# William-wAng618/roboticAttack

Hardware: AMD Instinct MI355X
Metric: attack-steps/sec (bs=64, 3x50x50 patch, OpenVLA-7B) (higher is better)
Workload: dtype bf16; 1 GPU; UADA_wrapper_ddp inner step: bs=64/rank (global 64), patch 3,50,50, geometry=True, maskidx=[0]; OpenVLA-7B shape, random init; u8 frames resident in HBM; global_batch=64, parallelism=dp1, regions=weak, visible_gpus=1, labelled_rows_per_rank=128, tunableop_entries_loaded_min_over_ranks=173

## Files before the change

### roboticattack_amd/csrc/vaa_attention.hip

```cpp
#include "vaa_common.h"

#include <cstdlib>
#include <mutex>

#include "../../include/vaa_model_ops.h"

namespace vaa {

typedef short v4s __attribute__((ext_vector_type(4)));
typedef short v8s __attribute__((ext_vector_type(8)));
typedef float v4f __attribute__((ext_vector_type(4)));
typedef __attribute__((address_space(3))) v4s* lds_v4s_ptr;

struct AttnStr {
    long b, t, h;
};

struct AttnFwdArgs {
    const uint16_t *q, *k, *v;
    uint16_t* o;
    float* lse;
    AttnStr sq, sk, sv, so;
    const int32_t* cu;
    int B, H, T, hd;
    float scale_log2;
};

struct SeqInfo {
    int T;
    long tok0;
    bool packed;
};
__device__ __forceinline__ SeqInfo seq_info(const int32_t* cu, int b, int Tmax) {
    SeqInfo si;
    si.packed = cu != nullptr;
    si.tok0 = si.packed ? cu[b] : 0;
    si.T = si.packed ? cu[b + 1] - cu[b] : Tmax;
    return si;
}
__device__ __forceinline__ long row_base(const AttnStr& st, const SeqInfo& si, int b, int h) {
    return (si.packed ? si.tok0 * st.t : (long)b * st.b) + (long)h * st.h;
}

constexpr int kTile = 64;

__device__ __forceinline__ float fast_exp2(float x) { return __builtin_amdgcn_exp2f(x); }

__device__ __forceinline__ v4s lds_tr16(const uint16_t* p) {
    return __builtin_amdgcn_ds_read_tr16_b64_v4i16((lds_v4s_ptr)(p));
}

__device__ __forceinline__ v8s cat8(v4s lo, v4s hi) { return __builtin_shufflevector(lo, hi, 0, 1, 2, 3, 4, 5, 6, 7); }

typedef __bf16 bf2 __attribute__((ext_vector_type(2)));
typedef float f2 __attribute__((ext_vector_type(2)));

__device__ __forceinline__ uint32_t cvt_pk_bf16(float lo, float hi) {
    const bf2 r = __builtin_convertvector((f2){lo, hi}, bf2);
    return *reinterpret_cast<const uint32_t*>(&r);
}

__device__ __forceinline__ v8s pack8(v4f a, v4f b) {
    uint4 r;
    r.x = cvt_pk_bf16(a[0], a[1]);
    r.y = cvt_pk_bf16(a[2], a[3]);
    r.z = cvt_pk_bf16(b[0], b[1]);
    r.w = cvt_pk_bf16(b[2], b[3]);
    return *reinterpret_cast<v8s*>(&r);
}

typedef unsigned int v4u __attribute__((ext_vector_type(4)));

__device__ __forceinline__ __amdgpu_buffer_rsrc_t slice_rsrc(const uint16_t* base, long st, int T, int hd) {
    return __builtin_amdgcn_make_buffer_rsrc((void*)base, 0, (int)((((long)T - 1) * st + hd) * 2), 0x00020000);
}

template <int HDP>
struct TileRegs {
    static constexpr int kChunks = kTile * (HDP / 8) / 256;
    v4u r[kChunks];
    __device__ __forceinline__ void load(__amdgpu_buffer_rsrc_t rs, int st_bytes, int row0) {
#pragma unroll
        for (int it = 0; it < kChunks; ++it) {
            const int ch = threadIdx.x + it * 256;
            const int row = ch / (HDP / 8), cc = ch % (HDP / 8);
            r[it] = __builtin_amdgcn_raw_buffer_load_b128(rs, (row0 + row) * st_bytes + cc * 16, 0, 0);
        }
    }
    __device__ __forceinline__ void store(uint16_t* lds, int stride) const {
#pragma unroll
        for (int it = 0; it < kChunks; ++it) {
            const int ch = threadIdx.x + it * 256;
            const int row = ch / (HDP / 8), cc = ch % (HDP / 8);
            *reinterpret_cast<v4u*>(lds + row * stride + cc * 8) = r[it];
        }
    }
};

__device__ __forceinline__ bool block_to_pair(int nblk, int npairs, int& pair, int& blk, bool late_first = true) {
    const int bid = blockIdx.x, xcd = bid & 7, slot = bid >> 3;
    pair = (slot / nblk) * 8 + xcd;
    blk = late_first ? nblk - 1 - (slot % nblk) : slot % nblk;
    return pair < npairs;
}

template <int KS, int NT, bool CAUSAL, int G>
__global__ __launch_bounds__(256) void attn_fwd_kernel(AttnFwdArgs a) {
    constexpr int HDP = KS * 32;
    constexpr int SK = HDP + 8;
    constexpr int SV = HDP + 16;
    constexpr int QB = kTile * G, QW = 16 * G;
    __shared__ __attribute__((aligned(16))) uint16_t sK[kTile * SK];
    __shared__ __attribute__((aligned(16))) uint16_t sV[kTile * SV];

    const int nqb = (a.T + QB - 1) / QB;
    int pair, qb;
    if (!block_to_pair(nqb, a.B * a.H, pair, qb)) return;
    const int b = pair / a.H, h = pair - b * a.H;
    const SeqInfo si = seq_info(a.cu, b, a.T);
    const int T = si.T;
    if (qb * QB >= T) return;
    const int tid = threadIdx.x, lane = tid & 63, wv = tid >> 6, c = lane & 15, g = lane >> 4;
    const int q0 = qb * QB + wv * QW;

    const uint16_t* qp = a.q + row_base(a.sq, si, b, h);
    const uint16_t* kp = a.k + row_base(a.sk, si, b, h);
    const uint16_t* vp = a.v + row_base(a.sv, si, b, h);

    v8s qf[G][KS];
#pragma unroll
    for (int j = 0; j < G; ++j) {
        const int q = q0 + 16 * j + c;
#pragma unroll
        for (int ks = 0; ks < KS; ++ks) {
            const int d0 = ks * 32 + g * 8;
            uint4 r = make_uint4(0, 0, 0, 0);
            if (q < T && d0 < a.hd) r = *reinterpret_cast<const uint4*>(qp + (long)q * a.sq.t + d0);
            qf[j][ks] = *reinterpret_cast<v8s*>(&r);
        }
    }

    const int kend = CAUSAL ? min(T, (qb + 1) * QB) : T;
    const int ntile = (kend + kTile - 1) / kTile;

    v4f acc[G][NT];
    float m[G], lsum[G];
#pragma unroll
    for (int j = 0; j < G; ++j) {
#pragma unroll
        for (int nt = 0; nt < NT; ++nt) acc[j][nt] = (v4f){0.f, 0.f, 0.f, 0.f};
        m[j] = -INFINITY;
        lsum[j] = 0.0f;
    }

    const __amdgpu_buffer_rsrc_t krs = slice_rsrc(kp, a.sk.t, T, a.hd), vrs = slice_rsrc(vp, a.sv.t, T, a.hd);
    const int kst = (int)a.sk.t * 2, vst = (int)a.sv.t * 2;
    TileRegs<HDP> rk, rv;
    rk.load(krs, kst, 0);
    rv.load(vrs, vst, 0);
    for (int kt = 0; kt < ntile; ++kt) {
        __syncthreads();
        rk.store(sK, SK);
        rv.store(sV, SV);
        __syncthreads();
        if (kt + 1 < ntile) {
            rk.load(krs, kst, (kt + 1) * kTile);
            rv.load(vrs, vst, (kt + 1) * kTile);
        }
        const int key0 = kt * kTile;
        if (CAUSAL && key0 > q0 + QW - 1) continue;

        v4f st[G][4];
#pragma unroll
        for (int rp = 0; rp < 2; ++rp) {
            v8s kfr[2][KS];
#pragma unroll
            for (int rl = 0; rl < 2; ++rl)
#pragma unroll
                for (int ks = 0; ks < KS; ++ks) kfr[rl][ks] = *reinterpret_cast<const v8s*>(&sK[((2 * rp + rl) * 16 + c) * SK + ks * 32 + g * 8]);
#pragma unroll
            for (int j = 0; j < G; ++j)
#pragma unroll
                for (int rl = 0; rl < 2; ++rl) {
                    v4f t = (v4f){0.f, 0.f, 0.f, 0.f};
#pragma unroll
                    for (int ks = 0; ks < KS; ++ks) t = __builtin_amdgcn_mfma_f32_16x16x32_bf16(kfr[rl][ks], qf[j][ks], t, 0, 0, 0);
                    st[j][2 * rp + rl] = t;
                }
        }
#pragma unroll
        for (int j = 0; j < G; ++j) {
            const int qj0 = q0 + 16 * j, q = qj0 + c;
            const bool need_mask = (key0 + kTile > T) || (CAUSAL && key0 + kTile - 1 > qj0);
            if (need_mask) {
#pragma unroll
                for (int rt = 0; rt < 4; ++rt)
#pragma unroll
                    for (int r = 0; r < 4; ++r) {
                        const int key = key0 + rt * 16 + g * 4 + r;
                        if (key >= T || (CAUSAL && key > q)) st[j][rt][r] = -INFINITY;
                    }
            }
            float mx = -INFINITY;
#pragma unroll
            for (int rt = 0; rt < 4; ++rt)
#pragma unroll
                for (int r = 0; r < 4; ++r) mx = fmaxf(mx, st[j][rt][r]);
            mx = fmaxf(mx, __shfl_xor(mx, 16, 64));
            mx = fmaxf(mx, __shfl_xor(mx, 32, 64));
            const float mn = fmaxf(m[j], mx * a.scale_log2);
            const float mu = (mn == -INFINITY) ? 0.0f : mn;
            const float alpha = fast_exp2(m[j] - mu);
            m[j] = mn;
            float ps = 0.0f;
#pragma unroll
            for (int rt = 0; rt < 4; ++rt)
#pragma unroll
                for (int r = 0; r < 4; ++r) {
                    const float p = fast_exp2(__builtin_fmaf(st[j][rt][r], a.scale_log2, -mu));
                    st[j][rt][r] = p;
                    ps += p;
                }
            lsum[j] = lsum[j] * alpha + ps;
#pragma unroll
            for (int nt = 0; nt < NT; ++nt) acc[j][nt] *= alpha;
        }
#pragma unroll
        for (int half = 0; half < 2; ++half) {
            const uint16_t* vrow = &sV[(half * 32 + 4 * g + (c >> 2)) * SV + (c & 3) * 4];
            v8s vfr[NT];
#pragma unroll
            for (int nt = 0; nt < NT; ++nt) vfr[nt] = cat8(lds_tr16(vrow + nt * 16), lds_tr16(vrow + 16 * SV + nt * 16));
#pragma unroll
            for (int j = 0; j < G; ++j) {
                const v8s pf = pack8(st[j][2 * half], st[j][2 * half + 1]);
#pragma unroll
                for (int nt = 0; nt < NT; ++nt) acc[j][nt] = __builtin_amdgcn_mfma_f32_16x16x32_bf16(vfr[nt], pf, acc[j][nt], 0, 0, 0);
            }
        }
    }
#pragma unroll
    for (int j = 0; j < G; ++j) {
        const int q = q0 + 16 * j + c;
        float ls = lsum[j];
        ls += __shfl_xor(ls, 16, 64);
        ls += __shfl_xor(ls, 32, 64);
        if (q < T) {
            const float inv = ls > 0.0f ? 1.0f / ls : 0.0f;
            uint16_t* op = a.o + row_base(a.so, si, b, h) + (long)q * a.so.t;
#pragma unroll
            for (int nt = 0; nt < NT; ++nt) {
                const int d0 = nt * 16 + g * 4;
                if (d0 < a.hd) {
                    uint2 w;
                    w.x = cvt_pk_bf16(acc[j][nt][0] * inv, acc[j][nt][1] * inv);
                    w.y = cvt_pk_bf16(acc[j][nt][2] * inv, acc[j][nt][3] * inv);
                    *reinterpret_cast<uint2*>(op + d0) = w;
                }
            }
            if (g == 0) a.lse[((long)b * a.H + h) * a.T + q] = (m[j] + __builtin_log2f(ls)) * 0.69314718055994531f;
        }
    }
}

struct AttnBwdArgs {
    const uint16_t *q, *k, *v, *o, *dout;
    const float* lse;
    float* dsum;
    uint16_t *dq, *dk, *dv;
    AttnStr sq, sk, sv, so, sdo, sdq, sdk, sdv;
    const int32_t* cu;
    const float *rope_cos, *rope_sin;
    int B, H, T, hd;
    float scale, scale_log2;
};

template <int NT>
__device__ __forceinline__ void store_grad_row(uint16_t* op, const v4f (&acc)[NT], float scale, int g, int hd, const float* cosr, const float* sinr) {
    if (cosr) {
#pragma unroll
        for (int nt = 0; nt < NT / 2; ++nt) {
            const int d0 = nt * 16 + g * 4;
            const float4 c4 = *reinterpret_cast<const float4*>(cosr + d0), s4 = *reinterpret_cast<const float4*>(sinr + d0);
            const float cs[4] = {c4.x, c4.y, c4.z, c4.w}, sn[4] = {s4.x, s4.y, s4.z, s4.w};
            float o1[4], o2[4];
#pragma unroll
            for (int r = 0; r < 4; ++r) {
                const float g1 = acc[nt][r] * scale, g2 = acc[nt + NT / 2][r] * scale;
                o1[r] = g1 * cs[r] + g2 * sn[r];
                o2[r] = g2 * cs[r] - g1 * sn[r];
            }
            uint2 w;
            w.x = cvt_pk_bf16(o1[0], o1[1]); w.y = cvt_pk_bf16(o1[2], o1[3]);
            *reinterpret_cast<uint2*>(op + d0) = w;
            w.x = cvt_pk_bf16(o2[0], o2[1]); w.y = cvt_pk_bf16(o2[2], o2[3]);
            *reinterpret_cast<uint2*>(op + d0 + NT * 8) = w;
        }
        return;
    }
#pragma unroll
    for (int nt = 0; nt < NT; ++nt) {
        const int d0 = nt * 16 + g * 4;
        if (d0 < hd) {
            uint2 w;
            w.x = cvt_pk_bf16(acc[nt][0] * scale, acc[nt][1] * scale);
            w.y = cvt_pk_bf16(acc[nt][2] * scale, acc[nt][3] * scale);
            *reinterpret_cast<uint2*>(op + d0) = w;
        }
    }
}

template <int KS>
__device__ __forceinline__ void load_row_frags(v8s (&f)[KS], const uint16_t* row, bool valid, int g, int hd) {
#pragma unroll
    for (int ks = 0; ks < KS; ++ks) {
        const int d0 = ks * 32 + g * 8;
        uint4 r = make_uint4(0, 0, 0, 0);
        if (valid && d0 < hd) r = *reinterpret_cast<const uint4*>(row + d0);
        f[ks] = *reinterpret_cast<v8s*>(&r);
    }
}

__device__ __forceinline__ float bf_lo(uint32_t w) { return __uint_as_float(w << 16); }
__device__ __forceinline__ float bf_hi(uint32_t w) { return __uint_as_float(w & 0xffff0000u); }

template <int KS>
__device__ __forceinline__ void load_tile_frags(v8s (&af)[KS], const uint16_t* tile, int stride, int rt, int c, int g) {
#pragma unroll
    for (int ks = 0; ks < KS; ++ks) af[ks] = *reinterpret_cast<const v8s*>(&tile[(rt * 16 + c) * stride + ks * 32 + g * 8]);
}
template <int KS>
__device__ __forceinline__ v4f frag_dot(const v8s (&af)[KS], const v8s (&bf)[KS]) {
    v4f acc = (v4f){0.f, 0.f, 0.f, 0.f};
#pragma unroll
    for (int ks = 0; ks < KS; ++ks) acc = __builtin_amdgcn_mfma_f32_16x16x32_bf16(af[ks], bf[ks], acc, 0, 0, 0);
    return acc;
}

template <int KS, int NT, bool CAUSAL, int G>
__global__ __launch_bounds__(256) void attn_bwd_dq_kernel(AttnBwdArgs a) {
    constexpr int HDP = KS * 32;
    constexpr int SK = HDP + 16, SV = HDP + 8;
    constexpr int QB = kTile * G, QW = 16 * G;
    __shared__ __attribute__((aligned(16))) uint16_t sK[kTile * SK];
    __shared__ __attribute__((aligned(16))) uint16_t sV[kTile * SV];

    const int nqb = (a.T + QB - 1) / QB;
    int pair, qb;
    if (!block_to_pair(nqb, a.B * a.H, pair, qb)) return;
    const int b = pair / a.H, h = pair - b * a.H;
    const SeqInfo si = seq_info(a.cu, b, a.T);
    const int T = si.T;
    if (qb * QB >= T) return;
    const int tid = threadIdx.x, lane = tid & 63, wv = tid >> 6, c = lane & 15, g = lane >> 4;
    const int q0 = qb * QB + wv * QW;

    const uint16_t* kp = a.k + row_base(a.sk, si, b, h);
    const uint16_t* vp = a.v + row_base(a.sv, si, b, h);
    v8s qf[G][KS], dof[G][KS];
    float Dq[G], lse2[G];
#pragma unroll
    for (int j = 0; j < G; ++j) {
        const int q = q0 + 16 * j + c;
        const bool qv = q < T;
        load_row_frags<KS>(qf[j], a.q + row_base(a.sq, si, b, h) + (long)q * a.sq.t, qv, g, a.hd);
        load_row_frags<KS>(dof[j], a.dout + row_base(a.sdo, si, b, h) + (long)q * a.sdo.t, qv, g, a.hd);
        float dq_ = 0.0f;
        v8s of[KS];
        load_row_frags<KS>(of, a.o + row_base(a.so, si, b, h) + (long)q * a.so.t, qv, g, a.hd);
#pragma unroll
        for (int ks = 0; ks < KS; ++ks)
#pragma unroll
            for (int e = 0; e < 8; ++e) dq_ += bf16_bits_to_f32((uint16_t)of[ks][e]) * bf16_bits_to_f32((uint16_t)dof[j][ks][e]);
        dq_ += __shfl_xor(dq_, 16, 64);
        dq_ += __shfl_xor(dq_, 32, 64);
        Dq[j] = dq_;
        const long rowid = ((long)b * a.H + h) * a.T + q;
        if (qv && g == 0) a.dsum[rowid] = dq_;
        lse2[j] = qv ? a.lse[rowid] * 1.4426950408889634f : INFINITY;
    }

    const int kend = CAUSAL ? min(T, (qb + 1) * QB) : T;
    const int ntile = (kend + kTile - 1) / kTile;
    v4f acc[G][NT];
#pragma unroll
    for (int j = 0; j < G; ++j)
#pragma unroll
        for (int nt = 0; nt < NT; ++nt) acc[j][nt] = (v4f){0.f, 0.f, 0.f, 0.f};

    const __amdgpu_buffer_rsrc_t krs = slice_rsrc(kp, a.sk.t, T, a.hd), vrs = slice_rsrc(vp, a.sv.t, T, a.hd);
    const int kst = (int)a.sk.t * 2, vst = (int)a.sv.t * 2;
    TileRegs<HDP> rk, rv;
    rk.load(krs, kst, 0);
    rv.load(vrs, vst, 0);
    for (int kt = 0; kt < ntile; ++kt) {
        __syncthreads();
        rk.store(sK, SK);
        rv.store(sV, SV);
        __syncthreads();
        if (kt + 1 < ntile) {
            rk.load(krs, kst, (kt + 1) * kTile);
            rv.load(vrs, vst, (kt + 1) * kTile);
        }
        const int key0 = kt * kTile;
        if (CAUSAL && key0 > q0 + QW - 1) continue;
        const bool need_mask = (key0 + kTile > T) || (CAUSAL && key0 + kTile - 1 > q0);
#pragma unroll
        for (int half = 0; half < 2; ++half) {
            if (CAUSAL && key0 + half * 32 > q0 + QW - 1) continue;
            v4f ds[G][2];
#pragma unroll
            for (int rl = 0; rl < 2; ++rl) {
                const int rt = 2 * half + rl;
                v8s ak[KS], av[KS];
                load_tile_frags<KS>(ak, sK, SK, rt, c, g);
                load_tile_frags<KS>(av, sV, SV, rt, c, g);
#pragma unroll
                for (int j = 0; j < G; ++j) {
                    const v4f st = frag_dot<KS>(ak, qf[j]);
                    const v4f dp = frag_dot<KS>(av, dof[j]);
                    const int q = q0 + 16 * j + c;
#pragma unroll
                    for (int r = 0; r < 4; ++r) {
                        float p = fast_exp2(__builtin_fmaf(st[r], a.scale_log2, -lse2[j]));
                        if (need_mask) {
                            const int key = key0 + rt * 16 + g * 4 + r;
                            if (key >= T || (CAUSAL && key > q)) p = 0.0f;
                        }
                        ds[j][rl][r] = p * (dp[r] - Dq[j]);
                    }
                }
            }
            const uint16_t* krow = &sK[(half * 32 + 4 * g + (c >> 2)) * SK + (c & 3) * 4];
            v8s kfr[NT];
#pragma unroll
            for (int nt = 0; nt < NT; ++nt) kfr[nt] = cat8(lds_tr16(krow + nt * 16), lds_tr16(krow + 16 * SK + nt * 16));
#pragma unroll
            for (int j = 0; j < G; ++j) {
                const v8s dsf = pack8(ds[j][0], ds[j][1]);
#pragma unroll
                for (int nt = 0; nt < NT; ++nt) acc[j][nt] = __builtin_amdgcn_mfma_f32_16x16x32_bf16(kfr[nt], dsf, acc[j][nt], 0, 0, 0);
            }
        }
    }
#pragma unroll
    for (int j = 0; j < G; ++j) {
        const int q = q0 + 16 * j + c;
        if (q < T) {
            const long ro = (si.tok0 + q) * (a.hd >> 1);
            store_grad_row<NT>(a.dq + row_base(a.sdq, si, b, h) + (long)q * a.sdq.t, acc[j], a.scale, g, a.hd,
                               a.rope_cos ? a.rope_cos + ro : nullptr, a.rope_cos ? a.rope_sin + ro : nullptr);
        }
    }
}

template <int KS, int NT, bool CAUSAL, int G>
__global__ __launch_bounds__(256) void attn_bwd_dkv_kernel(AttnBwdArgs a) {
    constexpr int HDP = KS * 32;
    constexpr int SQ = HDP + 16;
    constexpr int KB = kTile * G, KW = 16 * G;
    __shared__ __attribute__((aligned(16))) uint16_t sQ[kTile * SQ];
    __shared__ __attribute__((aligned(16))) uint16_t sDO[kTile * SQ];
    __shared__ float sL[kTile], sD[kTile];

    const int nkb = (a.T + KB - 1) / KB;
    int pair, kb;
    if (!block_to_pair(nkb, a.B * a.H, pair, kb, !CAUSAL)) return;
    const int b = pair / a.H, h = pair - b * a.H;
    const SeqInfo si = seq_info(a.cu, b, a.T);
    const int T = si.T;
    if (kb * KB >= T) return;
    const int tid = threadIdx.x, lane = tid & 63, wv = tid >> 6, c = lane & 15, g = lane >> 4;
    const int key0w = kb * KB + wv * KW;

    v8s kf[G][KS], vf[G][KS];
#pragma unroll
    for (int j = 0; j < G; ++j) {
        const int key = key0w + 16 * j + c;
        load_row_frags<KS>(kf[j], a.k + row_base(a.sk, si, b, h) + (long)key * a.sk.t, key < T, g, a.hd);
        load_row_frags<KS>(vf[j], a.v + row_base(a.sv, si, b, h) + (long)key * a.sv.t, key < T, g, a.hd);
    }
    const uint16_t* qp = a.q + row_base(a.sq, si, b, h);
    const uint16_t* dop = a.dout + row_base(a.sdo, si, b, h);
    const float* lsep = a.lse + ((long)b * a.H + h) * a.T;
    const float* dsp = a.dsum + ((long)b * a.H + h) * a.T;

    v4f dk[G][NT], dv[G][NT];
#pragma unroll
    for (int j = 0; j < G; ++j)
#pragma unroll
        for (int nt = 0; nt < NT; ++nt) {
            dk[j][nt] = (v4f){0.f, 0.f, 0.f, 0.f};
            dv[j][nt] = (v4f){0.f, 0.f, 0.f, 0.f};
        }
    const int nqt = (T + kTile - 1) / kTile;
    const int qt0 = CAUSAL ? kb * G : 0;
    TileRegs<HDP> rq, rdo;
    float rstat = 0.0f;
    auto load_stats = [&](int qbase) {
        if (tid < 128) {
            const int qq = qbase + (tid & 63);
            if (tid < 64) rstat = qq < T ? lsep[qq] * 1.4426950408889634f : INFINITY;
            else rstat = qq < T ? dsp[qq] : 0.0f;
        }
    };
    const __amdgpu_buffer_rsrc_t qrs = slice_rsrc(qp, a.sq.t, T, a.hd), dors = slice_rsrc(dop, a.sdo.t, T, a.hd);
    const int qst = (int)a.sq.t * 2, dost = (int)a.sdo.t * 2;
    rq.load(qrs, qst, qt0 * kTile);
    rdo.load(dors, dost, qt0 * kTile);
    load_stats(qt0 * kTile);
    for (int qt = qt0; qt < nqt; ++qt) {
        __syncthreads();
        rq.store(sQ, SQ);
        rdo.store(sDO, SQ);
        if (tid < 64) sL[tid] = rstat;
        else if (tid < 128) sD[tid - 64] = rstat;
        __syncthreads();
        if (qt + 1 < nqt) {
            rq.load(qrs, qst, (qt + 1) * kTile);
            rdo.load(dors, dost, (qt + 1) * kTile);
            load_stats((qt + 1) * kTile);
        }
        const int qb0 = qt * kTile;
        if (CAUSAL && qb0 + kTile - 1 < key0w) continue;
        const bool need_mask = CAUSAL && qb0 < key0w + KW - 1;
#pragma unroll
        for (int half = 0; half < 2; ++half) {
            if (CAUSAL && qb0 + half * 32 + 31 < key0w) continue;
            v4f p[G][2], ds[G][2];
#pragma unroll
            for (int rl = 0; rl < 2; ++rl) {
                const int rt = 2 * half + rl;
                v8s aq[KS], ado[KS];
                load_tile_frags<KS>(aq, sQ, SQ, rt, c, g);
                load_tile_frags<KS>(ado, sDO, SQ, rt, c, g);
#pragma unroll
                for (int j = 0; j < G; ++j) {
                    const v4f s = frag_dot<KS>(aq, kf[j]);
                    const v4f dp = frag_dot<KS>(ado, vf[j]);
                    const int key = key0w + 16 * j + c;
#pragma unroll
                    for (int r = 0; r < 4; ++r) {
                        const int ql = rt * 16 + g * 4 + r;
                        float pe = fast_exp2(__builtin_fmaf(s[r], a.scale_log2, -sL[ql]));
                        if (CAUSAL && need_mask && key > qb0 + ql) pe = 0.0f;
                        p[j][rl][r] = pe;
                        ds[j][rl][r] = pe * (dp[r] - sD[ql]);
                    }
                }
            }
            const int ro = (half * 32 + 4 * g + (c >> 2)) * SQ + (c & 3) * 4;
            {
                v8s fr[NT];
#pragma unroll
                for (int nt = 0; nt < NT; ++nt) fr[nt] = cat8(lds_tr16(&sDO[ro + nt * 16]), lds_tr16(&sDO[ro + 16 * SQ + nt * 16]));
#pragma unroll
                for (int j = 0; j < G; ++j) {
                    const v8s pf = pack8(p[j][0], p[j][1]);
#pragma unroll
                    for (int nt = 0; nt < NT; ++nt) dv[j][nt] = __builtin_amdgcn_mfma_f32_16x16x32_bf16(fr[nt], pf, dv[j][nt], 0, 0, 0);
                }
#pragma unroll
                for (int nt = 0; nt < NT; ++nt) fr[nt] = cat8(lds_tr16(&sQ[ro + nt * 16]), lds_tr16(&sQ[ro + 16 * SQ + nt * 16]));
#pragma unroll
                for (int j = 0; j < G; ++j) {
                    const v8s dsf = pack8(ds[j][0], ds[j][1]);
#pragma unroll
                    for (int nt = 0; nt < NT; ++nt) dk[j][nt] = __builtin_amdgcn_mfma_f32_16x16x32_bf16(fr[nt], dsf, dk[j][nt], 0, 0, 0);
                }
            }
        }
    }
#pragma unroll
    for (int j = 0; j < G; ++j) {
        const int key = key0w + 16 * j + c;
        if (key < T) {
            const long ro = (si.tok0 + key) * (a.hd >> 1);
            store_grad_row<NT>(a.dk + row_base(a.sdk, si, b, h) + (long)key * a.sdk.t, dk[j], a.scale, g, a.hd,
                               a.rope_cos ? a.rope_cos + ro : nullptr, a.rope_cos ? a.rope_sin + ro : nullptr);
            store_grad_row<NT>(a.dv + row_base(a.sdv, si, b, h) + (long)key * a.sdv.t, dv[j], 1.0f, g, a.hd, nullptr, nullptr);
        }
    }
}

static void attn_groups(int hd, int& gf, int& gq, int& gk) {
    static int cfg[3] = {0, 0, 0};
    static std::once_flag once;
    std::call_once(once, [] {
        const char* ev = getenv("VAA_ATTN_G");
        for (int i = 0; i < 3; ++i) cfg[i] = (ev && ev[0] && ev[1] && ev[2] && (ev[i] == '1' || ev[i] == '2')) ? ev[i] - '0' : 0;
    });
    const int dflt = (hd > 64 && hd <= 80) ? 2 : 1;
    gf = cfg[0] ? cfg[0] : dflt;
    gq = cfg[1] ? cfg[1] : dflt;
    gk = cfg[2] ? cfg[2] : dflt;
}

template <bool CAUSAL>
static int launch_bwd(const AttnBwdArgs& a, hipStream_t st) {
    int gf, gq, gk;
    attn_groups(a.hd, gf, gq, gk);
    const unsigned pairs8 = (unsigned)(((long)a.B * a.H + 7) / 8 * 8);
    const unsigned grid_q = pairs8 * (unsigned)((a.T + kTile * gq - 1) / (kTile * gq)), grid_k = pairs8 * (unsigned)((a.T + kTile * gk - 1) / (kTile * gk));
#define VAA_ATT_BWD(KS, NT)                                                                                                  \
    do {                                                                                                                     \
        if (gq == 2) hipLaunchKernelGGL((attn_bwd_dq_kernel<KS, NT, CAUSAL, 2>), dim3(grid_q), dim3(256), 0, st, a);         \
        else hipLaunchKernelGGL((attn_bwd_dq_kernel<KS, NT, CAUSAL, 1>), dim3(grid_q), dim3(256), 0, st, a);                 \
        int rc = check_launch("vaa_model_attention_bwd(dq)");                                                                \
        if (rc != VAA_OK) return rc;                                                                                         \
        if (gk == 2) hipLaunchKernelGGL((attn_bwd_dkv_kernel<KS, NT, CAUSAL, 2>), dim3(grid_k), dim3(256), 0, st, a);        \
        else hipLaunchKernelGGL((attn_bwd_dkv_kernel<KS, NT, CAUSAL, 1>), dim3(grid_k), dim3(256), 0, st, a);                \
        return check_launch("vaa_model_attention_bwd(dkv)");                                                                 \
    } while (0)
    if (a.hd <= 64) VAA_ATT_BWD(2, 4);
    else if (a.hd <= 80) VAA_ATT_BWD(3, 5);
    else if (a.hd <= 96) VAA_ATT_BWD(3, 6);
    else VAA_ATT_BWD(4, 8);
#undef VAA_ATT_BWD
}

template <bool CAUSAL>
static int launch_fwd(const AttnFwdArgs& a, hipStream_t st) {
    int gf, gq, gk;
    attn_groups(a.hd, gf, gq, gk);
    const unsigned grid = (unsigned)(((long)a.B * a.H + 7) / 8 * 8) * (unsigned)((a.T + kTile * gf - 1) / (kTile * gf));
#define VAA_ATT_FWD(KS, NT)                                                                                          \
    do {                                                                                                             \
        if (gf == 2) hipLaunchKernelGGL((attn_fwd_kernel<KS, NT, CAUSAL, 2>), dim3(grid), dim3(256), 0, st, a);      \
        else hipLaunchKernelGGL((attn_fwd_kernel<KS, NT, CAUSAL, 1>), dim3(grid), dim3(256), 0, st, a);              \
    } while (0)
    if (a.hd <= 64) VAA_ATT_FWD(2, 4);
    else if (a.hd <= 80) VAA_ATT_FWD(3, 5);
    else if (a.hd <= 96) VAA_ATT_FWD(3, 6);
    else VAA_ATT_FWD(4, 8);
#undef VAA_ATT_FWD
    return check_launch("vaa_model_attention_fwd");
}

static bool strides_ok(const int64_t* s) { return s && (s[0] % 8) == 0 && (s[1] % 8) == 0 && (s[2] % 8) == 0; }
static AttnStr mk(const int64_t* s) { AttnStr r; r.b = s[0]; r.t = s[1]; r.h = s[2]; return r; }

}

extern "C" int vaa_model_attention_fwd(const uint16_t* q, const int64_t* q_str, const uint16_t* k, const int64_t* k_str, const uint16_t* v,
                                       const int64_t* v_str, uint16_t* o, const int64_t* o_str, float* lse, const int32_t* cu_seqlens, int B,
                                       int H, int T, int hd, int causal, float scale, void* stream) {
    using namespace vaa;
    if (!q || !k || !v || !o || !lse) {
        set_error("vaa_model_attention_fwd: null pointer argument");
        return VAA_E_INVALID;
    }
    if (B <= 0 || H <= 0 || T <= 0 || hd <= 0 || hd > 128 || (hd % 8) != 0 || !strides_ok(q_str) || !strides_ok(k_str) || !strides_ok(v_str) ||
        !strides_ok(o_str)) {
        set_error("vaa_model_attention_fwd: unsupported shape (B=%d H=%d T=%d hd=%d; hd %% 8 == 0, hd <= 128, strides %% 8 == 0)", B, H, T, hd);
        return VAA_E_UNSUPPORTED;
    }
    AttnFwdArgs a;
    a.q = q; a.k = k; a.v = v; a.o = o; a.lse = lse;
    a.sq = mk(q_str); a.sk = mk(k_str); a.sv = mk(v_str); a.so = mk(o_str);
    a.cu = cu_seqlens;
    a.B = B; a.H = H; a.T = T; a.hd = hd;
    a.scale_log2 = scale * 1.4426950408889634f;
    return causal ? launch_fwd<true>(a, (hipStream_t)stream) : launch_fwd<false>(a, (hipStream_t)stream);
}

extern "C" int vaa_model_attention_bwd(const uint16_t* q, const int64_t* q_str, const uint16_t* k, const int64_t* k_str, const uint16_t* v,
                                       const int64_t* v_str, const uint16_t* o, const int64_t* o_str, const uint16_t* dout,
                                       const int64_t* do_str, const float* lse, float* dsum, uint16_t* dq, const int64_t* dq_str, uint16_t* dk,
                                       const int64_t* dk_str, uint16_t* dv, const int64_t* dv_str, const float* rope_cos, const float* rope_sin,
                                       const int32_t* cu_seqlens, int B, int H, int T, int hd, int causal, float scale, void* stream) {
    using namespace vaa;
    if (!q || !k || !v || !o || !dout || !lse || !dsum || !dq || !dk || !dv) {
        set_error("vaa_model_attention_bwd: null pointer argument");
        return VAA_E_INVALID;
    }
    if (B <= 0 || H <= 0 || T <= 0 || hd <= 0 || hd > 128 || (hd % 8) != 0 || !strides_ok(q_str) || !strides_ok(k_str) || !strides_ok(v_str) ||
        !strides_ok(o_str) || !strides_ok(do_str) || !strides_ok(dq_str) || !strides_ok(dk_str) || !strides_ok(dv_str)) {
        set_error("vaa_model_attention_bwd: unsupported shape (B=%d H=%d T=%d hd=%d; hd %% 8 == 0, hd <= 128, strides %% 8 == 0)", B, H, T, hd);
        return VAA_E_UNSUPPORTED;
    }
    AttnBwdArgs a;
    a.q = q; a.k = k; a.v = v; a.o = o; a.dout = dout; a.lse = lse; a.dsum = dsum; a.dq = dq; a.dk = dk; a.dv = dv;
    a.sq = mk(q_str); a.sk = mk(k_str); a.sv = mk(v_str); a.so = mk(o_str); a.sdo = mk(do_str);
    a.sdq = mk(dq_str); a.sdk = mk(dk_str); a.sdv = mk(dv_str);
    if ((rope_cos != nullptr) != (rope_sin != nullptr) || (rope_cos && hd != 64 && hd != 128)) {
        set_error("vaa_model_attention_bwd: fused rotary adjoint needs both tables and hd in {64, 128} (hd=%d)", hd);
        return VAA_E_UNSUPPORTED;
    }
    a.rope_cos = rope_cos; a.rope_sin = rope_sin;
    a.cu = cu_seqlens;
    a.B = B; a.H = H; a.T = T; a.hd = hd;
    a.scale = scale;
    a.scale_log2 = scale * 1.4426950408889634f;
    return causal ? launch_bwd<true>(a, (hipStream_t)stream) : launch_bwd<false>(a, (hipStream_t)stream);
}
```

Before: 2.151 attack-steps/s.

## Double-buffer LDS tiles in attention kernels and vectorize softmax math

Adds double-buffered LDS staging for K/V (forward, dQ) and Q/dO/stats (dKV) so each iteration needs one barrier instead of two, and the next tile's global load overlaps compute. This applies when head dim is at most 96, or always for the dKV kernel. It also replaces the shfl_xor row reductions with permlane16/32 swaps, precomputes a single mask limit per lane, and vectorizes the exp2/FMA work with packed f2 FMAs. The forward pass skips the accumulator rescale when no lane's running max changed. The cost is doubled LDS use, which can lower occupancy, plus extra code complexity.

```diff
diff --git a/roboticattack_amd/csrc/vaa_attention.hip b/roboticattack_amd/csrc/vaa_attention.hip
--- a/roboticattack_amd/csrc/vaa_attention.hip
+++ b/roboticattack_amd/csrc/vaa_attention.hip
@@ -46,6 +46,30 @@
 
 __device__ __forceinline__ float fast_exp2(float x) { return __builtin_amdgcn_exp2f(x); }
 
+typedef float f2 __attribute__((ext_vector_type(2)));
+
+__device__ __forceinline__ f2 fma2(f2 a, float s, float t) { return __builtin_elementwise_fma(a, (f2){s, s}, (f2){t, t}); }
+__device__ __forceinline__ v4f exp2_fma4(v4f x, float s, float t) {
+    const f2 lo = fma2((f2){x[0], x[1]}, s, t), hi = fma2((f2){x[2], x[3]}, s, t);
+    return (v4f){fast_exp2(lo[0]), fast_exp2(lo[1]), fast_exp2(hi[0]), fast_exp2(hi[1])};
+}
+
+__device__ __forceinline__ float rows_max(float x) {
+    auto r = __builtin_amdgcn_permlane16_swap(__float_as_uint(x), __float_as_uint(x), false, false);
+    x = fmaxf(__uint_as_float(r[0]), __uint_as_float(r[1]));
+    r = __builtin_amdgcn_permlane32_swap(__float_as_uint(x), __float_as_uint(x), false, false);
+    return fmaxf(__uint_as_float(r[0]), __uint_as_float(r[1]));
+}
+__device__ __forceinline__ float rows_sum(float x) {
+    auto r = __builtin_amdgcn_permlane16_swap(__float_as_uint(x), __float_as_uint(x), false, false);
+    x = __uint_as_float(r[0]) + __uint_as_float(r[1]);
+    r = __builtin_amdgcn_permlane32_swap(__float_as_uint(x), __float_as_uint(x), false, false);
+    return __uint_as_float(r[0]) + __uint_as_float(r[1]);
+}
+
+enum { kAttnFwd = 0, kAttnDq = 1, kAttnDkv = 2 };
+constexpr bool attn_double_buffer(int kernel, int hdp) { return hdp <= 96 || kernel == kAttnDkv; }
+
 __device__ __forceinline__ v4s lds_tr16(const uint16_t* p) {
     return __builtin_amdgcn_ds_read_tr16_b64_v4i16((lds_v4s_ptr)(p));
 }
@@ -53,7 +77,6 @@
 __device__ __forceinline__ v8s cat8(v4s lo, v4s hi) { return __builtin_shufflevector(lo, hi, 0, 1, 2, 3, 4, 5, 6, 7); }
 
 typedef __bf16 bf2 __attribute__((ext_vector_type(2)));
-typedef float f2 __attribute__((ext_vector_type(2)));
 
 __device__ __forceinline__ uint32_t cvt_pk_bf16(float lo, float hi) {
     const bf2 r = __builtin_convertvector((f2){lo, hi}, bf2);
@@ -110,8 +133,9 @@
     constexpr int SK = HDP + 8;
     constexpr int SV = HDP + 16;
     constexpr int QB = kTile * G, QW = 16 * G;
-    __shared__ __attribute__((aligned(16))) uint16_t sK[kTile * SK];
-    __shared__ __attribute__((aligned(16))) uint16_t sV[kTile * SV];
+    constexpr bool DB = attn_double_buffer(kAttnFwd, HDP);
+    __shared__ __attribute__((aligned(16))) uint16_t sK[(DB ? 2 : 1) * kTile * SK];
+    __shared__ __attribute__((aligned(16))) uint16_t sV[(DB ? 2 : 1) * kTile * SV];
 
     const int nqb = (a.T + QB - 1) / QB;
     int pair, qb;
@@ -158,15 +182,38 @@
     TileRegs<HDP> rk, rv;
     rk.load(krs, kst, 0);
     rv.load(vrs, vst, 0);
-    for (int kt = 0; kt < ntile; ++kt) {
-        __syncthreads();
+    if (DB) {
         rk.store(sK, SK);
         rv.store(sV, SV);
-        __syncthreads();
-        if (kt + 1 < ntile) {
-            rk.load(krs, kst, (kt + 1) * kTile);
-            rv.load(vrs, vst, (kt + 1) * kTile);
-        }
+        if (1 < ntile) {
+            rk.load(krs, kst, kTile);
+            rv.load(vrs, vst, kTile);
+        }
+    }
+    const int kfo = c * SK + g * 8, vfo = (4 * g + (c >> 2)) * SV + (c & 3) * 4;
+    for (int kt = 0; kt < ntile; ++kt) {
+        if (DB) {
+            __syncthreads();
+            if (kt + 1 < ntile) {
+                rk.store(sK + ((kt + 1) & 1) * (kTile * SK), SK);
+                rv.store(sV + ((kt + 1) & 1) * (kTile * SV), SV);
+                if (kt + 2 < ntile) {
+                    rk.load(krs, kst, (kt + 2) * kTile);
+                    rv.load(vrs, vst, (kt + 2) * kTile);
+                }
+            }
+        } else {
+            __syncthreads();
+            rk.store(sK, SK);
+            rv.store(sV, SV);
+            __syncthreads();
+            if (kt + 1 < ntile) {
+                rk.load(krs, kst, (kt + 1) * kTile);
+                rv.load(vrs, vst, (kt + 1) * kTile);
+            }
+        }
+        const uint16_t* tK = sK + (DB ? (kt & 1) * (kTile * SK) : 0) + kfo;
+        const uint16_t* tV = sV + (DB ? (kt & 1) * (kTile * SV) : 0) + vfo;
         const int key0 = kt * kTile;
         if (CAUSAL && key0 > q0 + QW - 1) continue;
 
@@ -177,7 +224,7 @@
 #pragma unroll
             for (int rl = 0; rl < 2; ++rl)
 #pragma unroll
-                for (int ks = 0; ks < KS; ++ks) kfr[rl][ks] = *reinterpret_cast<const v8s*>(&sK[((2 * rp + rl) * 16 + c) * SK + ks * 32 + g * 8]);
+                for (int ks = 0; ks < KS; ++ks) kfr[rl][ks] = *reinterpret_cast<const v8s*>(&tK[(2 * rp + rl) * 16 * SK + ks * 32]);
 #pragma unroll
             for (int j = 0; j < G; ++j)
 #pragma unroll
@@ -190,44 +237,44 @@
         }
 #pragma unroll
         for (int j = 0; j < G; ++j) {
-            const int qj0 = q0 + 16 * j, q = qj0 + c;
+            const int qj0 = q0 + 16 * j;
             const bool need_mask = (key0 + kTile > T) || (CAUSAL && key0 + kTile - 1 > qj0);
             if (need_mask) {
+                const int lim = (CAUSAL ? min(T - 1, qj0 + c) : T - 1) - key0 - g * 4;
 #pragma unroll
                 for (int rt = 0; rt < 4; ++rt)
 #pragma unroll
-                    for (int r = 0; r < 4; ++r) {
-                        const int key = key0 + rt * 16 + g * 4 + r;
-                        if (key >= T || (CAUSAL && key > q)) st[j][rt][r] = -INFINITY;
-                    }
+                    for (int r = 0; r < 4; ++r)
+                        if (rt * 16 + r > lim) st[j][rt][r] = -INFINITY;
             }
             float mx = -INFINITY;
 #pragma unroll
             for (int rt = 0; rt < 4; ++rt)
 #pragma unroll
                 for (int r = 0; r < 4; ++r) mx = fmaxf(mx, st[j][rt][r]);
-            mx = fmaxf(mx, __shfl_xor(mx, 16, 64));
-            mx = fmaxf(mx, __shfl_xor(mx, 32, 64));
+            mx = rows_max(mx);
             const float mn = fmaxf(m[j], mx * a.scale_log2);
             const float mu = (mn == -INFINITY) ? 0.0f : mn;
             const float alpha = fast_exp2(m[j] - mu);
+            const bool moved = __builtin_amdgcn_ballot_w64(mn != m[j]) != 0;
             m[j] = mn;
-            float ps = 0.0f;
-#pragma unroll
-            for (int rt = 0; rt < 4; ++rt)
-#pragma unroll
-                for (int r = 0; r < 4; ++r) {
-                    const float p = fast_exp2(__builtin_fmaf(st[j][rt][r], a.scale_log2, -mu));
-                    st[j][rt][r] = p;
-                    ps += p;
-                }
-            lsum[j] = lsum[j] * alpha + ps;
-#pragma unroll
-            for (int nt = 0; nt < NT; ++nt) acc[j][nt] *= alpha;
+            f2 ps2 = (f2){0.0f, 0.0f};
+#pragma unroll
+            for (int rt = 0; rt < 4; ++rt) {
+                const v4f p = exp2_fma4(st[j][rt], a.scale_log2, -mu);
+                st[j][rt] = p;
+                ps2 += (f2){p[0], p[1]};
+                ps2 += (f2){p[2], p[3]};
+            }
+            lsum[j] = lsum[j] * alpha + (ps2[0] + ps2[1]);
+            if (moved) {
+#pragma unroll
+                for (int nt = 0; nt < NT; ++nt) acc[j][nt] *= alpha;
+            }
         }
 #pragma unroll
         for (int half = 0; half < 2; ++half) {
-            const uint16_t* vrow = &sV[(half * 32 + 4 * g + (c >> 2)) * SV + (c & 3) * 4];
+            const uint16_t* vrow = tV + half * 32 * SV;
             v8s vfr[NT];
 #pragma unroll
             for (int nt = 0; nt < NT; ++nt) vfr[nt] = cat8(lds_tr16(vrow + nt * 16), lds_tr16(vrow + 16 * SV + nt * 16));
@@ -242,9 +289,7 @@
 #pragma unroll
     for (int j = 0; j < G; ++j) {
         const int q = q0 + 16 * j + c;
-        float ls = lsum[j];
-        ls += __shfl_xor(ls, 16, 64);
-        ls += __shfl_xor(ls, 32, 64);
+        const float ls = rows_sum(lsum[j]);
         if (q < T) {
             const float inv = ls > 0.0f ? 1.0f / ls : 0.0f;
             uint16_t* op = a.o + row_base(a.so, si, b, h) + (long)q * a.so.t;
@@ -342,8 +387,9 @@
     constexpr int HDP = KS * 32;
     constexpr int SK = HDP + 16, SV = HDP + 8;
     constexpr int QB = kTile * G, QW = 16 * G;
-    __shared__ __attribute__((aligned(16))) uint16_t sK[kTile * SK];
-    __shared__ __attribute__((aligned(16))) uint16_t sV[kTile * SV];
+    constexpr bool DB = attn_double_buffer(kAttnDq, HDP);
+    __shared__ __attribute__((aligned(16))) uint16_t sK[(DB ? 2 : 1) * kTile * SK];
+    __shared__ __attribute__((aligned(16))) uint16_t sV[(DB ? 2 : 1) * kTile * SV];
 
     const int nqb = (a.T + QB - 1) / QB;
     int pair, qb;
@@ -372,8 +418,7 @@
         for (int ks = 0; ks < KS; ++ks)
 #pragma unroll
             for (int e = 0; e < 8; ++e) dq_ += bf16_bits_to_f32((uint16_t)of[ks][e]) * bf16_bits_to_f32((uint16_t)dof[j][ks][e]);
-        dq_ += __shfl_xor(dq_, 16, 64);
-        dq_ += __shfl_xor(dq_, 32, 64);
+        dq_ = rows_sum(dq_);
         Dq[j] = dq_;
         const long rowid = ((long)b * a.H + h) * a.T + q;
         if (qv && g == 0) a.dsum[rowid] = dq_;
@@ -393,18 +438,43 @@
     TileRegs<HDP> rk, rv;
     rk.load(krs, kst, 0);
     rv.load(vrs, vst, 0);
-    for (int kt = 0; kt < ntile; ++kt) {
-        __syncthreads();
+    if (DB) {
         rk.store(sK, SK);
         rv.store(sV, SV);
-        __syncthreads();
-        if (kt + 1 < ntile) {
-            rk.load(krs, kst, (kt + 1) * kTile);
-            rv.load(vrs, vst, (kt + 1) * kTile);
-        }
+        if (1 < ntile) {
+            rk.load(krs, kst, kTile);
+            rv.load(vrs, vst, kTile);
+        }
+    }
+    for (int kt = 0; kt < ntile; ++kt) {
+        if (DB) {
+            __syncthreads();
+            if (kt + 1 < ntile) {
+                rk.store(sK + ((kt + 1) & 1) * (kTile * SK), SK);
+                rv.store(sV + ((kt + 1) & 1) * (kTile * SV), SV);
+                if (kt + 2 < ntile) {
+                    rk.load(krs, kst, (kt + 2) * kTile);
+                    rv.load(vrs, vst, (kt + 2) * kTile);
+                }
+            }
+        } else {
+            __syncthreads();
+            rk.store(sK, SK);
+            rv.store(sV, SV);
+            __syncthreads();
+            if (kt + 1 < ntile) {
+                rk.load(krs, kst, (kt + 1) * kTile);
+                rv.load(vrs, vst, (kt + 1) * kTile);
+            }
+        }
+        const uint16_t* tK = sK + (DB ? (kt & 1) * (kTile * SK) : 0);
+        const uint16_t* tV = sV + (DB ? (kt & 1) * (kTile * SV) : 0);
         const int key0 = kt * kTile;
         if (CAUSAL && key0 > q0 + QW - 1) continue;
         const bool need_mask = (key0 + kTile > T) || (CAUSAL && key0 + kTile - 1 > q0);
+        int lim[G];
+#pragma unroll
+        for (int j = 0; j < G; ++j) lim[j] = (CAUSAL ? min(T - 1, q0 + 16 * j + c) : T - 1) - key0 - g * 4;
 #pragma unroll
         for (int half = 0; half < 2; ++half) {
             if (CAUSAL && key0 + half * 32 > q0 + QW - 1) continue;
@@ -413,25 +483,22 @@
             for (int rl = 0; rl < 2; ++rl) {
                 const int rt = 2 * half + rl;
                 v8s ak[KS], av[KS];
-                load_tile_frags<KS>(ak, sK, SK, rt, c, g);
-                load_tile_frags<KS>(av, sV, SV, rt, c, g);
+                load_tile_frags<KS>(ak, tK, SK, rt, c, g);
+                load_tile_frags<KS>(av, tV, SV, rt, c, g);
 #pragma unroll
                 for (int j = 0; j < G; ++j) {
                     const v4f st = frag_dot<KS>(ak, qf[j]);
                     const v4f dp = frag_dot<KS>(av, dof[j]);
-                    const int q = q0 + 16 * j + c;
-#pragma unroll
-                    for (int r = 0; r < 4; ++r) {
-                        float p = fast_exp2(__builtin_fmaf(st[r], a.scale_log2, -lse2[j]));
-                        if (need_mask) {
-                            const int key = key0 + rt * 16 + g * 4 + r;
-                            if (key >= T || (CAUSAL && key > q)) p = 0.0f;
-                        }
-                        ds[j][rl][r] = p * (dp[r] - Dq[j]);
+                    v4f p = exp2_fma4(st, a.scale_log2, -lse2[j]);
+                    if (need_mask) {
+#pragma unroll
+                        for (int r = 0; r < 4; ++r)
+                            if (rt * 16 + r > lim[j]) p[r] = 0.0f;
                     }
+                    ds[j][rl] = p * (dp - Dq[j]);
                 }
             }
-            const uint16_t* krow = &sK[(half * 32 + 4 * g + (c >> 2)) * SK + (c & 3) * 4];
+            const uint16_t* krow = &tK[(half * 32 + 4 * g + (c >> 2)) * SK + (c & 3) * 4];
             v8s kfr[NT];
 #pragma unroll
             for (int nt = 0; nt < NT; ++nt) kfr[nt] = cat8(lds_tr16(krow + nt * 16), lds_tr16(krow + 16 * SK + nt * 16));
@@ -459,9 +526,10 @@
     constexpr int HDP = KS * 32;
     constexpr int SQ = HDP + 16;
     constexpr int KB = kTile * G, KW = 16 * G;
-    __shared__ __attribute__((aligned(16))) uint16_t sQ[kTile * SQ];
-    __shared__ __attribute__((aligned(16))) uint16_t sDO[kTile * SQ];
-    __shared__ float sL[kTile], sD[kTile];
+    constexpr bool DB = attn_double_buffer(kAttnDkv, HDP);
+    __shared__ __attribute__((aligned(16))) uint16_t sQ[(DB ? 2 : 1) * kTile * SQ];
+    __shared__ __attribute__((aligned(16))) uint16_t sDO[(DB ? 2 : 1) * kTile * SQ];
+    __shared__ __attribute__((aligned(16))) float sL[(DB ? 2 : 1) * kTile], sD[(DB ? 2 : 1) * kTile];
 
     const int nkb = (a.T + KB - 1) / KB;
     int pair, kb;
@@ -509,21 +577,45 @@
     rq.load(qrs, qst, qt0 * kTile);
     rdo.load(dors, dost, qt0 * kTile);
     load_stats(qt0 * kTile);
+    auto store_tile = [&](int buf) {
+        rq.store(sQ + buf * (kTile * SQ), SQ);
+        rdo.store(sDO + buf * (kTile * SQ), SQ);
+        if (tid < 64) sL[buf * kTile + tid] = rstat;
+        else if (tid < 128) sD[buf * kTile + tid - 64] = rstat;
+    };
+    auto load_tile = [&](int qt) {
+        rq.load(qrs, qst, qt * kTile);
+        rdo.load(dors, dost, qt * kTile);
+        load_stats(qt * kTile);
+    };
+    if (DB) {
+        store_tile(qt0 & 1);
+        if (qt0 + 1 < nqt) load_tile(qt0 + 1);
+    }
     for (int qt = qt0; qt < nqt; ++qt) {
-        __syncthreads();
-        rq.store(sQ, SQ);
-        rdo.store(sDO, SQ);
-        if (tid < 64) sL[tid] = rstat;
-        else if (tid < 128) sD[tid - 64] = rstat;
-        __syncthreads();
-        if (qt + 1 < nqt) {
-            rq.load(qrs, qst, (qt + 1) * kTile);
-            rdo.load(dors, dost, (qt + 1) * kTile);
-            load_stats((qt + 1) * kTile);
-        }
+        if (DB) {
+            __syncthreads();
+            if (qt + 1 < nqt) {
+                store_tile((qt + 1) & 1);
+                if (qt + 2 < nqt) load_tile(qt + 2);
+            }
+        } else {
+            __syncthreads();
+            store_tile(0);
+            __syncthreads();
+            if (qt + 1 < nqt) load_tile(qt + 1);
+        }
+        const int buf = DB ? (qt & 1) : 0;
+        const uint16_t* tQ = sQ + buf * (kTile * SQ);
+        const uint16_t* tDO = sDO + buf * (kTile * SQ);
+        const float* tL = sL + buf * kTile + g * 4;
+        const float* tD = sD + buf * kTile + g * 4;
         const int qb0 = qt * kTile;
         if (CAUSAL && qb0 + kTile - 1 < key0w) continue;
         const bool need_mask = CAUSAL && qb0 < key0w + KW - 1;
+        int lim[G];
+#pragma unroll
+        for (int j = 0; j < G; ++j) lim[j] = key0w + 16 * j + c - qb0 - g * 4;
 #pragma unroll
         for (int half = 0; half < 2; ++half) {
             if (CAUSAL && qb0 + half * 32 + 31 < key0w) continue;
@@ -532,28 +624,30 @@
             for (int rl = 0; rl < 2; ++rl) {
                 const int rt = 2 * half + rl;
                 v8s aq[KS], ado[KS];
-                load_tile_frags<KS>(aq, sQ, SQ, rt, c, g);
-                load_tile_frags<KS>(ado, sDO, SQ, rt, c, g);
+                load_tile_frags<KS>(aq, tQ, SQ, rt, c, g);
+                load_tile_frags<KS>(ado, tDO, SQ, rt, c, g);
+                const v4f l4 = *reinterpret_cast<const v4f*>(tL + rt * 16), d4 = *reinterpret_cast<const v4f*>(tD + rt * 16);
 #pragma unroll
                 for (int j = 0; j < G; ++j) {
                     const v4f s = frag_dot<KS>(aq, kf[j]);
                     const v4f dp = frag_dot<KS>(ado, vf[j]);
-                    const int key = key0w + 16 * j + c;
-#pragma unroll
-                    for (int r = 0; r < 4; ++r) {
-                        const int ql = rt * 16 + g * 4 + r;
-                        float pe = fast_exp2(__builtin_fmaf(s[r], a.scale_log2, -sL[ql]));
-                        if (CAUSAL && need_mask && key > qb0 + ql) pe = 0.0f;
-                        p[j][rl][r] = pe;
-                        ds[j][rl][r] = pe * (dp[r] - sD[ql]);
+                    const f2 lo = __builtin_elementwise_fma((f2){s[0], s[1]}, (f2){a.scale_log2, a.scale_log2}, (f2){-l4[0], -l4[1]});
+                    const f2 hi = __builtin_elementwise_fma((f2){s[2], s[3]}, (f2){a.scale_log2, a.scale_log2}, (f2){-l4[2], -l4[3]});
+                    v4f pe = (v4f){fast_exp2(lo[0]), fast_exp2(lo[1]), fast_exp2(hi[0]), fast_exp2(hi[1])};
+                    if (CAUSAL && need_mask) {
+#pragma unroll
+                        for (int r = 0; r < 4; ++r)
+                            if (rt * 16 + r < lim[j]) pe[r] = 0.0f;
                     }
+                    p[j][rl] = pe;
+                    ds[j][rl] = pe * (dp - d4);
                 }
             }
             const int ro = (half * 32 + 4 * g + (c >> 2)) * SQ + (c & 3) * 4;
             {
                 v8s fr[NT];
 #pragma unroll
-                for (int nt = 0; nt < NT; ++nt) fr[nt] = cat8(lds_tr16(&sDO[ro + nt * 16]), lds_tr16(&sDO[ro + 16 * SQ + nt * 16]));
+                for (int nt = 0; nt < NT; ++nt) fr[nt] = cat8(lds_tr16(&tDO[ro + nt * 16]), lds_tr16(&tDO[ro + 16 * SQ + nt * 16]));
 #pragma unroll
                 for (int j = 0; j < G; ++j) {
                     const v8s pf = pack8(p[j][0], p[j][1]);
@@ -561,7 +655,7 @@
                     for (int nt = 0; nt < NT; ++nt) dv[j][nt] = __builtin_amdgcn_mfma_f32_16x16x32_bf16(fr[nt], pf, dv[j][nt], 0, 0, 0);
                 }
 #pragma unroll
-                for (int nt = 0; nt < NT; ++nt) fr[nt] = cat8(lds_tr16(&sQ[ro + nt * 16]), lds_tr16(&sQ[ro + 16 * SQ + nt * 16]));
+                for (int nt = 0; nt < NT; ++nt) fr[nt] = cat8(lds_tr16(&tQ[ro + nt * 16]), lds_tr16(&tQ[ro + 16 * SQ + nt * 16]));
 #pragma unroll
                 for (int j = 0; j < G; ++j) {
                     const v8s dsf = pack8(ds[j][0], ds[j][1]);
```

New measurement: 2.152 attack-steps/s, median of 2. About the same (+0.0%).
